# MVPandey/DTS

Measured on AMD Instinct MI355X. Metric: scored_trajectories_per_sec, higher is better.
Workload: dtype bf16

## Files before the change

dts_amd/models/llama.py:

```python

from __future__ import annotations

import math
from typing import Optional

import torch
import torch.nn as nn
import torch.nn.functional as F

from dts_amd import ops
from dts_amd.models.config import ModelSpec
from dts_amd.ops.torch_ref import build_rope_cache
from dts_amd.parallel.tp import (
    ColumnParallelLinear,
    RowParallelLinear,
    TPContext,
    _init_weight,
)
from dts_amd.serving.batch import ForwardBatch


class LlamaAttention(nn.Module):
    def __init__(self, spec: ModelSpec, tp: TPContext, dtype):
        super().__init__()
        self.tp = tp
        assert spec.num_heads % tp.size == 0
        assert spec.num_kv_heads % tp.size == 0 or tp.size % spec.num_kv_heads == 0
        self.num_heads = spec.num_heads // tp.size
        self.num_kv_heads = max(1, spec.num_kv_heads // tp.size)
        self.head_dim = spec.head_dim
        self.scale = 1.0 / math.sqrt(spec.head_dim)
        q_out = self.num_heads * self.head_dim * tp.size
        kv_out = self.num_kv_heads * self.head_dim * tp.size
        self.qkv_proj = ColumnParallelLinear(
            spec.hidden_size, q_out + 2 * kv_out, tp, dtype=dtype
        )
        self.o_proj = RowParallelLinear(
            self.num_heads * self.head_dim * tp.size, spec.hidden_size, tp, dtype=dtype
        )
        self.q_size = self.num_heads * self.head_dim
        self.kv_size = self.num_kv_heads * self.head_dim

    def forward(
        self,
        hidden: torch.Tensor,
        batch: ForwardBatch,
        kv_layer: tuple,
        rope: tuple,
    ) -> torch.Tensor:
        T = hidden.shape[0]
        qkv = self.qkv_proj(hidden)
        q, k, v = qkv.split([self.q_size, self.kv_size, self.kv_size], dim=-1)
        q = q.view(T, self.num_heads, self.head_dim)
        k = k.view(T, self.num_kv_heads, self.head_dim)
        v = v.view(T, self.num_kv_heads, self.head_dim)

        k_cache, v_cache = kv_layer
        cos, sin = rope
        q, k = ops.rope_kv_append(
            q, k, v, batch.positions, cos, sin, k_cache, v_cache, batch.slot_mapping
        )

        out = torch.empty(q.shape, dtype=q.dtype, device=q.device)
        np_tok = batch.num_prefill_tokens
        if batch.num_prefill_seqs:
            ops.attn_prefill_paged(
                q[:np_tok],
                batch.cu_q,
                batch.positions[:np_tok],
                k_cache,
                v_cache,
                batch.prefill_block_tables,
                batch.prefill_kv_lens,
                self.scale,
                out=out[:np_tok],
            )
        if batch.num_decode_seqs:
            ops.attn_decode_paged(
                q[np_tok:],
                k_cache,
                v_cache,
                batch.decode_block_tables,
                batch.decode_kv_lens,
                self.scale,
                out=out[np_tok:],
            )
        return self.o_proj(out.reshape(T, -1))


class LlamaMLP(nn.Module):
    def __init__(self, spec: ModelSpec, tp: TPContext, dtype):
        super().__init__()
        self.gate_up_proj = ColumnParallelLinear(
            spec.hidden_size, 2 * spec.intermediate_size, tp, dtype=dtype
# ... 132 lines not shown
```

dts_amd/ops/__init__.py:

```python

from __future__ import annotations

import os

import torch

from dts_amd.ops import torch_ref
from dts_amd.utils.logging import logger

_hip = None
_hip_load_error: Exception | None = None


def _try_load_hip():
    global _hip, _hip_load_error
    if _hip is not None or _hip_load_error is not None:
        return _hip
    try:
        from dts_amd.ops import _hip_ext_loader

        _hip = _hip_ext_loader.load()
        logger.info("HIP extension loaded: %s", _hip.__name__)
    except Exception as e:
        _hip_load_error = e
# ... 31 lines not shown
            ext.rmsnorm(out, x, weight, eps)
            return out
    return torch_ref.rmsnorm(x, weight, eps)


def fused_add_rmsnorm(x, residual, weight, eps=1e-5):
    if _on_gpu(x):
        ext = _require_hip()
        if ext is not None:
            ext.fused_add_rmsnorm(x, residual, weight, eps)
            return x, residual
    return torch_ref.fused_add_rmsnorm(x, residual, weight, eps)


def layernorm(x, weight, bias, eps=1e-5):
    if _on_gpu(x):
        ext = _require_hip()
        if ext is not None:
            out = torch.empty_like(x)
            ext.layernorm(out, x, weight, bias, eps)
            return out
    return torch_ref.layernorm(x, weight, bias, eps)


def rope_kv_append(q, k, v, positions, cos, sin, k_cache, v_cache, slot_mapping):
    if _on_gpu(q):
        ext = _require_hip()
        if ext is not None:
            ext.rope_kv_append(q, k, v, positions, cos, sin, k_cache, v_cache, slot_mapping)
            return q, k
    q, k = torch_ref.rope_apply(q, k, positions, cos, sin)
    torch_ref.kv_append(k, v, k_cache, v_cache, slot_mapping)
    return q, k


def kv_append(k, v, k_cache, v_cache, slot_mapping):
    if _on_gpu(k):
        ext = _require_hip()
        if ext is not None:
            ext.kv_append(k, v, k_cache, v_cache, slot_mapping)
            return
    torch_ref.kv_append(k, v, k_cache, v_cache, slot_mapping)


def attn_prefill_paged(
    q, cu_q, q_positions, k_cache, v_cache, block_tables, kv_lens, scale=None,
    out=None,
):
    if _on_gpu(q):
        ext = _require_hip()
        if ext is not None:
            import math

            if out is None or not out.is_contiguous():
                out = torch.empty(q.shape, dtype=q.dtype, device=q.device)
            ext.attn_prefill_paged(
                out, q, cu_q, q_positions, k_cache, v_cache, block_tables, kv_lens,
                scale if scale is not None else 1.0 / math.sqrt(q.shape[-1]),
            )
            return out
    ref = torch_ref.attn_prefill_paged(
        q, cu_q, q_positions, k_cache, v_cache, block_tables, kv_lens, scale
    )
    if out is not None:
        out.copy_(ref)
        return out
# ... 198 lines not shown
```

dts_amd/ops/hip/attention.hip:

```cpp

#include "common.h"
#include "kv_cache.h"
#include <torch/extension.h>
#include <c10/hip/HIPStream.h>
#include <unordered_map>
#include <array>
#include <cstdlib>

using bf16x8 = __attribute__((ext_vector_type(8))) short;
using f32x4 = __attribute__((ext_vector_type(4))) float;
using f32x2 = __attribute__((ext_vector_type(2))) float;
using bf16x2 = __attribute__((ext_vector_type(2))) __bf16;
using u32x2 = __attribute__((ext_vector_type(2))) unsigned int;
using u32x4 = __attribute__((ext_vector_type(4))) unsigned int;


DEV bf16x8 kv_deq8(u32x2 w) {
  union { bf16x2 p[4]; bf16x8 v; } c;
  c.p[0] = __builtin_amdgcn_cvt_scalef32_pk_bf16_fp8(w[0], 1.0f, false);
  c.p[1] = __builtin_amdgcn_cvt_scalef32_pk_bf16_fp8(w[0], 1.0f, true);
  c.p[2] = __builtin_amdgcn_cvt_scalef32_pk_bf16_fp8(w[1], 1.0f, false);
  c.p[3] = __builtin_amdgcn_cvt_scalef32_pk_bf16_fp8(w[1], 1.0f, true);
  return c.v;
}


template <int G, int D, typename KV = short>
__global__ void __launch_bounds__(256)
attn_decode_kernel(float* __restrict__ ws_m,
                   float* __restrict__ ws_l,
                   float* __restrict__ ws_o,
                   const short* __restrict__ q,
                   const KV* __restrict__ kcache,
                   const KV* __restrict__ vcache,
                   const int* __restrict__ block_tables,
                   const int* __restrict__ kv_lens,
                   int max_blocks, int Hkv, float scale, long q_tstride) {
  constexpr int BS = 16;
  constexpr int NWAVE = 4;
  constexpr int LPK = 4;
  constexpr int DPL = D / LPK;
  constexpr int DPV = D / WAVE;
  const int seq = blockIdx.x;
  const int kvh = blockIdx.y;
  const int split = blockIdx.z;
  const int S = gridDim.z;
  const int Hq = Hkv * G;
  const int wave = threadIdx.x / WAVE;
  const int lane = threadIdx.x & (WAVE - 1);
  const int kv_len = kv_lens[seq];
  const int n_pages = (kv_len + BS - 1) / BS;
  const int pages_per_split = (n_pages + S - 1) / S;
  const int page_lo = split * pages_per_split;
  const int page_hi = min(n_pages, page_lo + pages_per_split);
  const long ws_base = (((long)seq * Hkv + kvh) * S + split) * G;
  if (page_lo >= page_hi) {
    for (int g = threadIdx.x; g < G; g += blockDim.x) {
      ws_m[ws_base + g] = -1e30f;
      ws_l[ws_base + g] = 0.f;
    }
    return;
  }

  __shared__ float s_scores[NWAVE][G][BS];
  __shared__ float s_m[NWAVE][G], s_l[NWAVE][G];
  __shared__ float s_o[NWAVE][G][D];

  const int c = lane & (LPK - 1);
  const int key_of_lane = lane / LPK;
  int qp_[G][DPL / 2];
#pragma unroll
  for (int g = 0; g < G; ++g) {
    const short* qp = q + (long)seq * q_tstride + (long)(kvh * G + g) * D + c * DPL;
#pragma unroll
    for (int i = 0; i < DPL / 2; ++i) qp_[g][i] = ((const int*)qp)[i];
  }

  float m[G], lsum[G], o[G][DPV];
#pragma unroll
  for (int g = 0; g < G; ++g) {
    m[g] = -1e30f;
    lsum[g] = 0.f;
#pragma unroll
    for (int d = 0; d < DPV; ++d) o[g][d] = 0.f;
  }

  const int* bt = block_tables + (long)seq * max_blocks;

  for (int page = page_lo + wave; page < page_hi; page += NWAVE) {
    const long blk = bt[page];
    const KV* kbase =
        kcache + ((blk * Hkv + kvh) * BS) * (long)D;
    const KV* vbase =
// ... 121 lines not shown
  for (int g = 0; g < G; ++g) {
    if (lane == 0) {
      s_m[wave][g] = m[g];
      s_l[wave][g] = lsum[g];
    }
#pragma unroll
    for (int d = 0; d < DPV; ++d) s_o[wave][g][lane * DPV + d] = o[g][d];
  }
  __syncthreads();

  const int tid = threadIdx.x;
  for (int gd = tid; gd < G * (D / 2); gd += blockDim.x) {
    const int g = gd / (D / 2);
    const int d0 = (gd % (D / 2)) * 2;
    float m_star = -1e30f;
#pragma unroll
    for (int w = 0; w < NWAVE; ++w) m_star = fmaxf(m_star, s_m[w][g]);
    float l_star = 0.f, acc0 = 0.f, acc1 = 0.f;
#pragma unroll
    for (int w = 0; w < NWAVE; ++w) {
      float f = (s_m[w][g] > -1e30f) ? __expf(s_m[w][g] - m_star) : 0.f;
      l_star += s_l[w][g] * f;
      acc0 += s_o[w][g][d0] * f;
      acc1 += s_o[w][g][d0 + 1] * f;
    }
    if (d0 == 0) {
      ws_m[ws_base + g] = m_star;
      ws_l[ws_base + g] = l_star;
    }
    float* wo = ws_o + (ws_base + g) * D;
    wo[d0] = acc0;
    wo[d0 + 1] = acc1;
  }
}

template <int D>
__global__ void __launch_bounds__(256)
attn_decode_combine(short* __restrict__ out,
                    const float* __restrict__ ws_m,
                    const float* __restrict__ ws_l,
                    const float* __restrict__ ws_o,
                    int S, int G, int Hkv) {
  const int seq = blockIdx.x;
  const int hq = blockIdx.y;
  const int kvh = hq / G;
  const int g = hq % G;
  const int Hq = Hkv * G;
  const long base0 = (((long)seq * Hkv + kvh) * S) * G + g;

  __shared__ float sh_f[64];
  __shared__ float sh_linv[1];
  if (threadIdx.x == 0) {
    float m_star = -1e30f;
    for (int s2 = 0; s2 < S; ++s2)
      m_star = fmaxf(m_star, ws_m[base0 + (long)s2 * G]);
    float l_star = 0.f;
    for (int s2 = 0; s2 < S; ++s2) {
      float mm = ws_m[base0 + (long)s2 * G];
      float f = (mm > -1e30f) ? __expf(mm - m_star) : 0.f;
      sh_f[s2] = f;
      l_star += ws_l[base0 + (long)s2 * G] * f;
    }
    sh_linv[0] = (l_star > 0.f) ? 1.f / l_star : 0.f;
  }
  __syncthreads();
  const float linv = sh_linv[0];
// ... 695 lines not shown
    }
    __syncthreads();
  }

  {
    float invl[4];
#pragma unroll
    for (int i = 0; i < 4; ++i) {
      float l = s_rowl[wave][(lane >> 4) * 4 + i];
      invl[i] = (l > 0.f) ? 1.f / l : 0.f;
    }
#pragma unroll
    for (int ct = 0; ct < CTILES; ++ct) {
#pragma unroll
      for (int i = 0; i < 4; ++i) {
        const int row = (lane >> 4) * 4 + i;
        const int row_global = wave * 16 + row;
        const int pos_local = tile * POS_PER_WG + row_global / G;
        if (pos_local >= q_len) continue;
        const int head = row_global % G;
        const int tok = q_start + pos_local;
        const int dim = ct * 16 + (lane & 15);
        out[((long)tok * Hq + kvh * G + head) * D + dim] =
            f2bf(o_acc[ct][i] * invl[i]);
      }
    }
  }
}


void attn_decode_paged(torch::Tensor out, torch::Tensor q,
                       torch::Tensor kcache, torch::Tensor vcache,
                       torch::Tensor block_tables, torch::Tensor kv_lens,
                       double scale) {
  const int B = q.size(0), Hq = q.size(1), D = q.size(2);
  const int Hkv = kcache.size(1);
  const int G = Hq / Hkv;
  const int max_blocks = block_tables.size(1);
  TORCH_CHECK(kcache.size(2) == 16, "block_size must be 16");
  const bool fp8 = kv_cache_is_fp8(kcache, vcache);
  TORCH_CHECK(block_tables.scalar_type() == torch::kInt32);
  TORCH_CHECK(q.stride(2) == 1 && q.stride(1) == D, "q heads must be dense");
  TORCH_CHECK(out.is_contiguous(), "out must be contiguous");
  const long q_tstride = q.stride(0);
  static const int S = [] {
    const char* e = getenv("DTS_DECODE_SPLITS");
    int v = e ? atoi(e) : 8;
    return (v >= 1 && v <= 64) ? v : 8;
  }();
  static std::unordered_map<std::string, std::array<torch::Tensor, 3>> ws_cache;
  const std::string key = std::to_string(q.get_device()) + ":" +
                          std::to_string(B) + ":" + std::to_string(Hkv) + ":" +
                          std::to_string(G) + ":" + std::to_string(D);
  auto it = ws_cache.find(key);
  if (it == ws_cache.end()) {
    auto f32 =
        torch::TensorOptions().dtype(torch::kFloat32).device(q.device());
    it = ws_cache
             .emplace(key,
                      std::array<torch::Tensor, 3>{
                          torch::empty({B, Hkv, S, G}, f32),
                          torch::empty({B, Hkv, S, G}, f32),
                          torch::empty({(long)B, Hkv, S, G, D}, f32)})
             .first;
  }
  torch::Tensor ws_m = it->second[0];
  torch::Tensor ws_l = it->second[1];
  torch::Tensor ws_o = it->second[2];
  dim3 grid(B, Hkv, S);
  dim3 block(256);
  auto stream = c10::hip::getCurrentHIPStream();
#define DECODE_LAUNCH(g, d, kv)                                              \
  hipLaunchKernelGGL((attn_decode_kernel<g, d, kv>), grid, block, 0, stream, \
                     (float*)ws_m.data_ptr(), (float*)ws_l.data_ptr(),       \
                     (float*)ws_o.data_ptr(), (const short*)q.data_ptr(),    \
                     (const kv*)kcache.data_ptr(),                           \
                     (const kv*)vcache.data_ptr(),                           \
                     (const int*)block_tables.data_ptr(),                    \
                     (const int*)kv_lens.data_ptr(), max_blocks, Hkv,        \
                     (float)scale, q_tstride)
#define DECODE_CASE(g, d)                                                    \
  do {                                                                       \
    if (fp8) DECODE_LAUNCH(g, d, unsigned char);                             \
    else DECODE_LAUNCH(g, d, short);                                         \
    hipLaunchKernelGGL((attn_decode_combine<d>), dim3(B, Hq), dim3(256), 0,  \
                       stream, (short*)out.data_ptr(),                       \
                       (const float*)ws_m.data_ptr(),                        \
                       (const float*)ws_l.data_ptr(),                        \
                       (const float*)ws_o.data_ptr(), S, G, Hkv);            \
  } while (0)
  if (D == 128 && G == 4) DECODE_CASE(4, 128);
  else if (D == 128 && G == 8) DECODE_CASE(8, 128);
  else if (D == 128 && G == 1) DECODE_CASE(1, 128);
  else if (D == 64 && G == 1) DECODE_CASE(1, 64);
  else TORCH_CHECK(false, "unsupported decode attn shape D=", D, " G=", G);
#undef DECODE_CASE
#undef DECODE_LAUNCH
  HIP_CHECK_LAST();
}

void attn_prefill_paged(torch::Tensor out, torch::Tensor q, torch::Tensor cu_q,
                        torch::Tensor q_pos, torch::Tensor kcache,
                        torch::Tensor vcache, torch::Tensor block_tables,
                        torch::Tensor kv_lens, double scale, int64_t swz) {
  if (swz < 0) {
    static int env_v = [] {
      const char* e = getenv("DTS_PREFILL_V");
      return e ? atoi(e) : -1;
    }();
    swz = (env_v >= 0) ? env_v : 5;
  }
  const bool fp8 = kv_cache_is_fp8(kcache, vcache);
  TORCH_CHECK(!fp8 || swz == 0 || swz == 4 || swz == 5,
              "prefill variant ", swz, " (DTS_PREFILL_V) does not support an "
              "FP8 KV cache; use 0, 4 or 5");
  const int Hq = q.size(1), D = q.size(2);
  const int Hkv = kcache.size(1);
// ... 121 lines not shown
```

dts_amd/ops/hip/bindings.cpp:

```cpp
#include <torch/extension.h>

void rmsnorm(torch::Tensor out, torch::Tensor x, torch::Tensor w, double eps);
void fused_add_rmsnorm(torch::Tensor x, torch::Tensor residual,
                       torch::Tensor w, double eps);
void silu_mul(torch::Tensor out, torch::Tensor in);
void layernorm(torch::Tensor out, torch::Tensor x, torch::Tensor w,
               torch::Tensor b, double eps);
void rope_kv_append(torch::Tensor q, torch::Tensor k, torch::Tensor v,
                    torch::Tensor positions, torch::Tensor cos_t,
                    torch::Tensor sin_t, torch::Tensor k_cache,
                    torch::Tensor v_cache, torch::Tensor slots);
void kv_append(torch::Tensor k, torch::Tensor v, torch::Tensor k_cache,
               torch::Tensor v_cache, torch::Tensor slots);
void attn_decode_paged(torch::Tensor out, torch::Tensor q,
                       torch::Tensor kcache, torch::Tensor vcache,
                       torch::Tensor block_tables, torch::Tensor kv_lens,
                       double scale);
void attn_prefill_paged(torch::Tensor out, torch::Tensor q, torch::Tensor cu_q,
                        torch::Tensor q_pos, torch::Tensor kcache,
                        torch::Tensor vcache, torch::Tensor block_tables,
                        torch::Tensor kv_lens, double scale, int64_t swz);
void top_p_sample(torch::Tensor out, torch::Tensor logits, torch::Tensor temps,
                  torch::Tensor top_ps, torch::Tensor seeds);
void derive_seeds(torch::Tensor out, torch::Tensor bases,
                  torch::Tensor positions);
void top_p_sample_v2(torch::Tensor out, torch::Tensor logits,
                     torch::Tensor temps, torch::Tensor top_ps,
                     torch::Tensor seeds, torch::Tensor ws_max,
                     torch::Tensor ws_bins, torch::Tensor ws_slice,
                     torch::Tensor ws_tau);
void gemv_bf16(torch::Tensor out, torch::Tensor x, torch::Tensor w);
void gemm_skinny_bf16(torch::Tensor out, torch::Tensor x, torch::Tensor w,
                      int64_t tiles_per_wg, int64_t unroll);
void gemm_skinny_swiglu_bf16(torch::Tensor out, torch::Tensor x,
                             torch::Tensor w);
void moe_grouped_linear(torch::Tensor out, torch::Tensor x, torch::Tensor w,
                        torch::Tensor counts, torch::Tensor offsets);
void gemm_skinny_w8_bf16(torch::Tensor out, torch::Tensor x, torch::Tensor w_q,
                         torch::Tensor scale, int64_t tiles_per_wg,
                         int64_t unroll);
void gemm_skinny_swiglu_w8_bf16(torch::Tensor out, torch::Tensor x,
                                torch::Tensor w_q, torch::Tensor scale);

PYBIND11_MODULE(TORCH_EXTENSION_NAME, m) {
  m.def("rmsnorm", &rmsnorm, "RMSNorm (bf16, CDNA4)");
  m.def("fused_add_rmsnorm", &fused_add_rmsnorm,
        "fused residual add + RMSNorm (in-place, bf16)");
  m.def("silu_mul", &silu_mul, "SwiGLU activation (bf16)");
  m.def("layernorm", &layernorm, "LayerNorm (bf16, GPT-2 path)");
  m.def("rope_kv_append", &rope_kv_append,
        "fused rotate-half RoPE + paged KV append (bf16 q/k/v; bf16 or FP8 "
        "e4m3fn cache)");
  m.def("kv_append", &kv_append,
        "paged KV append without RoPE (bf16 k/v; bf16 or FP8 e4m3fn cache)");
  m.def("attn_decode_paged", &attn_decode_paged,
        "paged GQA decode attention (bf16 q/out, bf16 or FP8 e4m3fn cache)");
  m.def("attn_prefill_paged", &attn_prefill_paged,
        "paged causal prefill attention (bf16 MFMA; bf16 or FP8 e4m3fn cache)",
        py::arg("out"), py::arg("q"), py::arg("cu_q"), py::arg("q_pos"),
        py::arg("kcache"), py::arg("vcache"), py::arg("block_tables"),
        py::arg("kv_lens"),
        py::arg("scale"), py::arg("swz") = -1);
  m.def("top_p_sample", &top_p_sample,
        "fused temperature softmax + top-p sampling (sort-free)");
  m.def("derive_seeds", &derive_seeds,
        "stateless (seed, position) mix for chained decode");
  m.def("top_p_sample_v2", &top_p_sample_v2,
        "gridded top-p sampler (vocab sliced across workgroups)");
  m.def("gemv_bf16", &gemv_bf16,
        "skinny-batch (M<=8) bf16 weight-streaming GEMV");
  m.def("gemm_skinny_bf16", &gemm_skinny_bf16,
        "skinny-M (M<=16) bf16 MFMA weight-streaming GEMM; tiles_per_wg "
        "pins the N-tiles per workgroup (1/2/4), unroll the k-chunks in "
        "flight (4/8; 8 needs K % 1024 == 0); 0 = auto",
        py::arg("out"), py::arg("x"), py::arg("w"),
        py::arg("tiles_per_wg") = 0, py::arg("unroll") = 0);
  m.def("gemm_skinny_swiglu_bf16", &gemm_skinny_swiglu_bf16,
        "skinny-M gate_up GEMM with fused SwiGLU epilogue: "
        "out[M,I] = silu(x Wg^T) * (x Wu^T), w = [Wg; Wu]");
  m.def("moe_grouped_linear", &moe_grouped_linear,
        "grouped per-expert skinny GEMM (capture-safe MoE decode)");
  m.def("gemm_skinny_w8_bf16", &gemm_skinny_w8_bf16,
        "W8A16 skinny-M (M<=16) GEMM: FP8 e4m3fn weights [N,K] with an fp32 "
        "per-row scale [N], bf16 x/out, fp32 accumulation; tiles_per_wg and "
        "unroll as for gemm_skinny_bf16",
        py::arg("out"), py::arg("x"), py::arg("w_q"), py::arg("scale"),
        py::arg("tiles_per_wg") = 0, py::arg("unroll") = 0);
  m.def("gemm_skinny_swiglu_w8_bf16", &gemm_skinny_swiglu_w8_bf16,
        "W8A16 gate_up GEMM with fused SwiGLU epilogue: w_q = [Wg; Wu], "
        "gate rows scale by scale[n], up rows by scale[I+n]");
}
```

dts_amd/ops/hip/common.h:

```cpp
#pragma once

#include <hip/hip_runtime.h>
#include <hip/hip_bf16.h>
#include <hip/hip_fp16.h>

#define WAVE 64
#define DEV __device__ __forceinline__

typedef __attribute__((ext_vector_type(4))) short short4v;
typedef __attribute__((ext_vector_type(8))) short short8v;
typedef __attribute__((ext_vector_type(4))) float float4v;

DEV float bf2f(short u) {
  union { float f; unsigned int i; } c;
  c.i = ((unsigned int)(unsigned short)u) << 16;
  return c.f;
}

DEV short f2bf(float f) {
  union { float f; unsigned int i; } c;
  c.f = f;
  unsigned int lsb = (c.i >> 16) & 1;
  c.i += 0x7fff + lsb;
  return (short)(c.i >> 16);
}

DEV short swiglu_bf16(short gate, short up) {
  float gf = bf2f(gate);
  float s = gf / (1.f + __expf(-gf));
  return f2bf(s * bf2f(up));
}

DEV float wave_sum(float v) {
#pragma unroll
  for (int off = 32; off > 0; off >>= 1) v += __shfl_xor(v, off, 64);
  return v;
}

DEV float wave_max(float v) {
#pragma unroll
  for (int off = 32; off > 0; off >>= 1) v = fmaxf(v, __shfl_xor(v, off, 64));
  return v;
}

#define HIP_CHECK_LAST()                                                      \
  do {                                                                        \
    hipError_t e = hipGetLastError();                                         \
    if (e != hipSuccess) {                                                    \
      TORCH_CHECK(false, "HIP kernel launch failed: ", hipGetErrorString(e)); \
    }                                                                         \
  } while (0)
```

dts_amd/ops/hip/elementwise.hip:

```cpp

#include "common.h"
#include "kv_cache.h"
#include <torch/extension.h>
#include <c10/hip/HIPStream.h>


template <int BLOCK>
__global__ void rmsnorm_kernel(short* __restrict__ out,
                               const short* __restrict__ x,
                               const short* __restrict__ w, float eps, int T,
                               int H) {
  __shared__ float red[BLOCK / WAVE];
  for (int row = blockIdx.x; row < T; row += gridDim.x) {
    const short* xr = x + (long)row * H;
    short* yr = out + (long)row * H;
    float ss = 0.f;
    for (int i = threadIdx.x * 8; i < H; i += BLOCK * 8) {
      short8v v = *(const short8v*)(xr + i);
#pragma unroll
      for (int j = 0; j < 8; ++j) {
        float f = bf2f(v[j]);
        ss += f * f;
      }
    }
// ... 124 lines not shown
    short8v g = *(const short8v*)(in + t * 2 * I + i);
    short8v u = *(const short8v*)(in + t * 2 * I + I + i);
    short8v o;
#pragma unroll
    for (int j = 0; j < 8; ++j) o[j] = swiglu_bf16(g[j], u[j]);
    *(short8v*)(out + t * I + i) = o;
  }
}


template <typename KV>
__global__ void rope_kv_append_kernel(
    short* __restrict__ q, short* __restrict__ k, const short* __restrict__ v,
    const long* __restrict__ positions, const float* __restrict__ cos_t,
    const float* __restrict__ sin_t, KV* __restrict__ k_cache,
    KV* __restrict__ v_cache, const long* __restrict__ slots, int T, int Hq,
    int Hk, int D, int BS, long cache_head_stride, long cache_block_stride,
    int do_rope, long q_tstride, long k_tstride, long v_tstride) {
  int unit = blockIdx.x * (blockDim.x / WAVE) + threadIdx.x / WAVE;
  int lane = threadIdx.x & (WAVE - 1);
  int units = T * (Hq + 2 * Hk);
  if (unit >= units) return;
  int t = unit / (Hq + 2 * Hk);
  int h = unit % (Hq + 2 * Hk);
  long pos = positions[t];
  int half = D / 2;

  if (do_rope && h < Hq + Hk) {
    short* base = (h < Hq) ? q + (long)t * q_tstride + (long)h * D
                           : k + (long)t * k_tstride + (long)(h - Hq) * D;
    for (int i = lane; i < half; i += WAVE) {
      float c = cos_t[pos * half + i];
      float s = sin_t[pos * half + i];
      float x1 = bf2f(base[i]);
      float x2 = bf2f(base[i + half]);
      base[i] = f2bf(x1 * c - x2 * s);
      base[i + half] = f2bf(x2 * c + x1 * s);
    }
  }
  if (h >= Hq) {
    bool is_v = h >= Hq + Hk;
    int kvh = is_v ? (h - Hq - Hk) : (h - Hq);
    const short* src = is_v ? v + (long)t * v_tstride + (long)kvh * D
                            : k + (long)t * k_tstride + (long)kvh * D;
    KV* cache = is_v ? v_cache : k_cache;
    long slot = slots[t];
    long block = slot / BS, off = slot % BS;
    KV* dst = cache + block * cache_block_stride + kvh * cache_head_stride +
              off * D;
    if constexpr (sizeof(KV) == 1) {
      for (int i = lane * 4; i < D; i += WAVE * 4) {
        int w0 = *(const int*)(src + i);
        int w1 = *(const int*)(src + i + 2);
        auto sat = [](int u) {
          return fminf(fmaxf(bf2f((short)(u & 0xffff)), -448.f), 448.f);
        };
        float f0 = sat(w0), f1 = sat(w0 >> 16);
        float f2 = sat(w1), f3 = sat(w1 >> 16);
        int codes = __builtin_amdgcn_cvt_pk_fp8_f32(f0, f1, 0, false);
        codes = __builtin_amdgcn_cvt_pk_fp8_f32(f2, f3, codes, true);
        *(int*)(dst + i) = codes;
      }
    } else {
      for (int i = lane * 2; i < D; i += WAVE * 2) {
        *(int*)(dst + i) = *(const int*)(src + i);
      }
    }
  }
}

// ... 114 lines not shown
```

dts_amd/ops/hip/gemm_skinny.hip:

```cpp

#include "common.h"
#include <torch/extension.h>
#include <c10/hip/HIPStream.h>

using bf16x8 = __attribute__((ext_vector_type(8))) short;
using f32x4 = __attribute__((ext_vector_type(4))) float;

#define NWAVES 4
#define KSTEP 32
#define KUNROLL 4

template <int KU, int NT, bool SWIGLU>
__global__ void __launch_bounds__(NWAVES* WAVE)
gemm_skinny_kernel(short* __restrict__ out,
                   const short* __restrict__ x,
                   const short* __restrict__ w,
                   int M, int N, int K, long x_ts, long out_ts,
                   int wg_stride, int tile_stride) {
  static_assert(!SWIGLU || NT == 2, "SwiGLU pairs one gate and one up tile");
  const int wave = threadIdx.x / WAVE;
  const int lane = threadIdx.x & (WAVE - 1);
  const int n0 = blockIdx.x * wg_stride;

  const int kq = K / NWAVES;
  const int kbeg = wave * kq;
  const int kend = kbeg + kq;

  const int a_row = lane & 15;
  const int k_off = (lane >> 4) * 8;
  const bool a_live = a_row < M;
  const short* xrow = x + (long)a_row * x_ts;
  bool b_live[NT];
  const short* wrow[NT];
#pragma unroll
  for (int j = 0; j < NT; ++j) {
    const int b_row = n0 + j * tile_stride + (lane & 15);
    b_live[j] = b_row < N;
    wrow[j] = w + (long)(b_live[j] ? b_row : 0) * K;
  }

  f32x4 acc[NT];
#pragma unroll
  for (int j = 0; j < NT; ++j) acc[j] = {0.f, 0.f, 0.f, 0.f};
  const bf16x8 zero8 = {0, 0, 0, 0, 0, 0, 0, 0};

  auto load_group = [&](int k0, bf16x8 (&a)[KU], bf16x8 (&b)[NT][KU]) {
#pragma unroll
    for (int u = 0; u < KU; ++u) {
      const int kk = k0 + u * KSTEP + k_off;
      a[u] = a_live ? *(const bf16x8*)(xrow + kk) : zero8;
#pragma unroll
      for (int j = 0; j < NT; ++j)
        b[j][u] = b_live[j] ? *(const bf16x8*)(wrow[j] + kk) : zero8;
    }
  };
// ... 1 lines not shown
#pragma unroll
    for (int u = 0; u < KU; ++u)
#pragma unroll
      for (int j = 0; j < NT; ++j)
        acc[j] = __builtin_amdgcn_mfma_f32_16x16x32_bf16(a[u], b[j][u], acc[j],
                                                         0, 0, 0);
  };
  for (int k0 = kbeg; k0 < kend; k0 += KSTEP * KU) {
    bf16x8 a[KU], b[NT][KU];
    load_group(k0, a, b);
    mfma_group(a, b);
  }

  __shared__ float red[NT][NWAVES][16][16];
  const int c_col = lane & 15;
#pragma unroll
  for (int j = 0; j < NT; ++j)
#pragma unroll
    for (int i = 0; i < 4; ++i)
      red[j][wave][(lane >> 4) * 4 + i][c_col] = acc[j][i];
  __syncthreads();
  if constexpr (SWIGLU) {
    if (wave == 0) {
#pragma unroll
      for (int i = 0; i < 4; ++i) {
        const int m = (lane >> 4) * 4 + i;
        const int n = n0 + c_col;
        if (m < M && n < tile_stride) {
          float g = red[0][0][m][c_col] + red[0][1][m][c_col] +
                    red[0][2][m][c_col] + red[0][3][m][c_col];
          float u = red[1][0][m][c_col] + red[1][1][m][c_col] +
                    red[1][2][m][c_col] + red[1][3][m][c_col];
          out[(long)m * out_ts + n] = swiglu_bf16(f2bf(g), f2bf(u));
        }
      }
    }
  } else {
    for (int j = wave; j < NT; j += NWAVES) {
#pragma unroll
      for (int i = 0; i < 4; ++i) {
        const int m = (lane >> 4) * 4 + i;
        const int n = n0 + j * tile_stride + c_col;
        if (m < M && n < N) {
          float v = red[j][0][m][c_col] + red[j][1][m][c_col] +
                    red[j][2][m][c_col] + red[j][3][m][c_col];
          out[(long)m * out_ts + n] = f2bf(v);
        }
      }
    }
  }
}


__global__ void __launch_bounds__(NWAVES* WAVE)
moe_grouped_kernel(short* __restrict__ out,
                   const short* __restrict__ x,
                   const short* __restrict__ w,
                   const int* __restrict__ counts,
                   const int* __restrict__ offsets,
                   int N, int K) {
  const int wave = threadIdx.x / WAVE;
  const int lane = threadIdx.x & (WAVE - 1);
  const int n0 = blockIdx.x * 16;
  const int e = blockIdx.y;
  const int cnt = counts[e];
  if (cnt == 0) return;
// ... 49 lines not shown
}

void moe_grouped_linear(torch::Tensor out, torch::Tensor x, torch::Tensor w,
                        torch::Tensor counts, torch::Tensor offsets) {
  TORCH_CHECK(x.scalar_type() == torch::kBFloat16 && x.is_contiguous());
  TORCH_CHECK(w.is_contiguous(), "expert weights must be contiguous [E,N,K]");
  TORCH_CHECK(out.is_contiguous());
  TORCH_CHECK(counts.scalar_type() == torch::kInt32 &&
              offsets.scalar_type() == torch::kInt32);
  const int K = x.size(1), E = w.size(0), N = w.size(1);
  TORCH_CHECK(K % (NWAVES * KSTEP * KUNROLL) == 0, "K must be /512");
  const int tiles = (N + 15) / 16;
  hipLaunchKernelGGL(moe_grouped_kernel, dim3(tiles, E), dim3(NWAVES * WAVE),
                     0, c10::hip::getCurrentHIPStream(),
                     (short*)out.data_ptr(), (const short*)x.data_ptr(),
                     (const short*)w.data_ptr(),
                     (const int*)counts.data_ptr(),
                     (const int*)offsets.data_ptr(), N, K);
  HIP_CHECK_LAST();
}

static int skinny_unroll(int K, int64_t unroll) {
  static const int env_ku = [] {
    const char* e = getenv("DTS_SKINNY_UNROLL");
    return (e && e[0] == '8') ? 8 : (e && e[0] == '4') ? 4 : 0;
  }();
  TORCH_CHECK(unroll != 8 || K % (NWAVES * KSTEP * 8) == 0,
              "unroll=8 needs K % 1024 == 0, got K=", K);
  int ku = unroll ? (int)unroll : env_ku ? env_ku : (K >= 8192 ? 8 : 4);
  if (K % (NWAVES * KSTEP * 8) != 0) ku = 4;
  return ku;
}

#define SKINNY_LAUNCH(KU_, NT_, SW_, grid_, wgs_, ts_)                        \
  hipLaunchKernelGGL((gemm_skinny_kernel<KU_, NT_, SW_>), dim3(grid_),       \
                     dim3(NWAVES * WAVE), 0, stream, (short*)out.data_ptr(), \
                     (const short*)x.data_ptr(), (const short*)w.data_ptr(), \
                     M, N, K, x.stride(0), out.stride(0), wgs_, ts_)

static int skinny_auto_tiles(int M, int tiles) {
  if (M < 8) return 1;
  if (tiles >= 4096) return 4;
  if (tiles >= 1024) return M > 8 ? 4 : 1;
  if (tiles >= 384) return 2;
  return 1;
}

void gemm_skinny_bf16(torch::Tensor out, torch::Tensor x, torch::Tensor w,
                      int64_t tiles_per_wg, int64_t unroll) {
  TORCH_CHECK(x.scalar_type() == torch::kBFloat16);
  TORCH_CHECK(w.is_contiguous(), "weight must be contiguous [N, K]");
  TORCH_CHECK(x.stride(1) == 1, "x rows must be dense");
  TORCH_CHECK(out.stride(1) == 1);
  const int M = x.size(0), K = x.size(1), N = w.size(0);
  TORCH_CHECK(M >= 1 && M <= 16, "skinny path is for M<=16");
  TORCH_CHECK(K % (NWAVES * KSTEP * KUNROLL) == 0, "K must be /512");
  TORCH_CHECK(w.size(1) == K && out.size(0) == M && out.size(1) == N);
  TORCH_CHECK(tiles_per_wg == 0 || tiles_per_wg == 1 || tiles_per_wg == 2 ||
                  tiles_per_wg == 4,
              "tiles_per_wg must be 0 (auto), 1, 2 or 4");
  TORCH_CHECK(unroll == 0 || unroll == 4 || unroll == 8,
              "unroll must be 0 (auto), 4 or 8");
  const int tiles = (N + 15) / 16;
  const int nt =
      tiles_per_wg ? (int)tiles_per_wg : skinny_auto_tiles(M, tiles);
  const int grid = (tiles + nt - 1) / nt;
  auto stream = c10::hip::getCurrentHIPStream();
  if (skinny_unroll(K, unroll) == 8) {
    if (nt == 4) SKINNY_LAUNCH(8, 4, false, grid, 64, 16);
    else if (nt == 2) SKINNY_LAUNCH(8, 2, false, grid, 32, 16);
    else SKINNY_LAUNCH(8, 1, false, grid, 16, 16);
  } else {
    if (nt == 4) SKINNY_LAUNCH(4, 4, false, grid, 64, 16);
    else if (nt == 2) SKINNY_LAUNCH(4, 2, false, grid, 32, 16);
    else SKINNY_LAUNCH(4, 1, false, grid, 16, 16);
  }
  HIP_CHECK_LAST();
}

void gemm_skinny_swiglu_bf16(torch::Tensor out, torch::Tensor x,
                             torch::Tensor w) {
  TORCH_CHECK(x.scalar_type() == torch::kBFloat16);
  TORCH_CHECK(w.is_contiguous(), "weight must be contiguous [2I, K]");
  TORCH_CHECK(x.stride(1) == 1, "x rows must be dense");
  TORCH_CHECK(out.stride(1) == 1);
  const int M = x.size(0), K = x.size(1), N = w.size(0);
  const int I = N / 2;
  TORCH_CHECK(M >= 1 && M <= 16, "skinny path is for M<=16");
  TORCH_CHECK(K % (NWAVES * KSTEP * KUNROLL) == 0, "K must be /512");
  TORCH_CHECK(N == 2 * I && I % 16 == 0, "fused SwiGLU needs I % 16 == 0");
  TORCH_CHECK(w.size(1) == K && out.size(0) == M && out.size(1) == I);
  const int grid = I / 16;
  auto stream = c10::hip::getCurrentHIPStream();
  if (skinny_unroll(K, 0) == 8)
    SKINNY_LAUNCH(8, 2, true, grid, 16, I);
  else
    SKINNY_LAUNCH(4, 2, true, grid, 16, I);
  HIP_CHECK_LAST();
}
#undef SKINNY_LAUNCH
```

Before: 0.3880.

## Fuse QKV skinny GEMM with RoPE and paged KV append; add optional in-launch decode combine

For pure-decode batches with head_dim 128 and a bf16 cache, the QKV projection now runs a skinny GEMM variant whose epilogue applies rotate-half RoPE and writes K/V straight into the paged cache. This removes the separate rope_kv_append launch and its re-read of the qkv output. The change also adds an opt-in mode, off by default and enabled via an env var, that folds the split-KV decode combine into the decode kernel using an atomic ticket. The fused GEMM tiles heads as 128-wide pairs of 16-column tiles, so grid shape and per-block work differ from the plain skinny path.

```diff
diff --git a/dts_amd/models/llama.py b/dts_amd/models/llama.py
--- a/dts_amd/models/llama.py
+++ b/dts_amd/models/llama.py
@@ -49,17 +49,34 @@
         rope: tuple,
     ) -> torch.Tensor:
         T = hidden.shape[0]
-        qkv = self.qkv_proj(hidden)
+        k_cache, v_cache = kv_layer
+        cos, sin = rope
+        proj = self.qkv_proj
+        fused = (
+            proj.bias is None
+            and proj.weight_q is None
+            and not proj.gather_output
+            and ops.qkv_rope_fusable(
+                hidden, proj.weight, k_cache, self.num_heads, self.num_kv_heads,
+                self.head_dim, pure_decode=batch.num_prefill_seqs == 0,
+            )
+        )
+        if fused:
+            qkv = ops.linear_qkv_rope_append(
+                hidden, proj.weight, batch.positions, cos, sin, k_cache, v_cache,
+                batch.slot_mapping, self.num_heads, self.num_kv_heads,
+            )
+        else:
+            qkv = proj(hidden)
         q, k, v = qkv.split([self.q_size, self.kv_size, self.kv_size], dim=-1)
         q = q.view(T, self.num_heads, self.head_dim)
         k = k.view(T, self.num_kv_heads, self.head_dim)
         v = v.view(T, self.num_kv_heads, self.head_dim)
-
-        k_cache, v_cache = kv_layer
-        cos, sin = rope
-        q, k = ops.rope_kv_append(
-            q, k, v, batch.positions, cos, sin, k_cache, v_cache, batch.slot_mapping
-        )
+        if not fused:
+            q, k = ops.rope_kv_append(
+                q, k, v, batch.positions, cos, sin, k_cache, v_cache,
+                batch.slot_mapping,
+            )
 
         out = torch.empty(q.shape, dtype=q.dtype, device=q.device)
         np_tok = batch.num_prefill_tokens
diff --git a/dts_amd/ops/__init__.py b/dts_amd/ops/__init__.py
--- a/dts_amd/ops/__init__.py
+++ b/dts_amd/ops/__init__.py
@@ -87,6 +87,37 @@
     q, k = torch_ref.rope_apply(q, k, positions, cos, sin)
     torch_ref.kv_append(k, v, k_cache, v_cache, slot_mapping)
     return q, k
+
+
+def qkv_rope_fusable(
+    x, weight, k_cache, num_heads, num_kv_heads, head_dim, pure_decode=True
+) -> bool:
+    return (
+        pure_decode
+        and head_dim == 128
+        and os.environ.get("DTS_FUSED_QKV_ROPE") != "0"
+        and _skinny_kind(x, weight) == "skinny"
+        and weight.dtype == torch.bfloat16
+        and weight.is_contiguous()
+        and weight.shape[0] == (num_heads + 2 * num_kv_heads) * head_dim
+        and k_cache.dtype == torch.bfloat16
+        and hip_available()
+    )
+
+
+def linear_qkv_rope_append(
+    x, weight, positions, cos, sin, k_cache, v_cache, slot_mapping,
+    num_heads, num_kv_heads,
+):
+    ext = _require_hip()
+    if ext is None:
+        raise RuntimeError("linear_qkv_rope_append needs the HIP extension")
+    out = torch.empty((x.shape[0], weight.shape[0]), dtype=x.dtype, device=x.device)
+    ext.gemm_skinny_qkv_rope_append(
+        out, x, weight, positions, cos, sin, k_cache, v_cache, slot_mapping,
+        num_heads, num_kv_heads,
+    )
+    return out
 
 
 def kv_append(k, v, k_cache, v_cache, slot_mapping):
diff --git a/dts_amd/ops/hip/attention.hip b/dts_amd/ops/hip/attention.hip
--- a/dts_amd/ops/hip/attention.hip
+++ b/dts_amd/ops/hip/attention.hip
@@ -25,7 +25,87 @@
 }
 
 
-template <int G, int D, typename KV = short>
+template <int G, int D>
+DEV void decode_combine_tail(short* out,
+                             float* ws_m,
+                             float* ws_l, float* ws_o, int* cnt, int seq,
+                             int kvh, int Hkv, int S) {
+  __shared__ float t_f[G][64];
+  __shared__ float t_l[G][64];
+  __shared__ float t_linv[G];
+  __shared__ int t_last;
+  const int tid = threadIdx.x;
+  asm volatile("s_waitcnt vmcnt(0)" ::: "memory");
+  __syncthreads();
+  if (tid == 0) {
+    int* c = cnt + (long)seq * Hkv + kvh;
+    __builtin_amdgcn_fence(__ATOMIC_RELEASE, "agent");
+    asm volatile("s_waitcnt vmcnt(0)" ::: "memory");
+    const int ticket = __hip_atomic_fetch_add(c, 1, __ATOMIC_RELAXED,
+                                              __HIP_MEMORY_SCOPE_AGENT);
+    const int last = ticket == S - 1;
+    if (last) {
+      __hip_atomic_store(c, 0, __ATOMIC_RELAXED, __HIP_MEMORY_SCOPE_AGENT);
+      __builtin_amdgcn_fence(__ATOMIC_ACQUIRE, "agent");
+      asm volatile("s_waitcnt vmcnt(0)" ::: "memory");
+    }
+    t_last = last;
+  }
+  __syncthreads();
+  if (!t_last) return;
+
+  const long base0 = (((long)seq * Hkv + kvh) * S) * G;
+  for (int i = tid; i < S * G; i += blockDim.x) {
+    t_f[i % G][i / G] = ws_m[base0 + i];
+    t_l[i % G][i / G] = ws_l[base0 + i];
+  }
+  __syncthreads();
+  if (tid < G) {
+    const int g = tid;
+    float m_star = -1e30f;
+    for (int s2 = 0; s2 < S; ++s2) m_star = fmaxf(m_star, t_f[g][s2]);
+    float l_star = 0.f;
+    for (int s2 = 0; s2 < S; ++s2) {
+      float mm = t_f[g][s2];
+      float f = (mm > -1e30f) ? __expf(mm - m_star) : 0.f;
+      t_f[g][s2] = f;
+      l_star += t_l[g][s2] * f;
+    }
+    t_linv[g] = (l_star > 0.f) ? 1.f / l_star : 0.f;
+  }
+  __syncthreads();
+  const int Hq = Hkv * G;
+#pragma unroll 1
+  for (int it = tid; it < G * (D / 4); it += blockDim.x) {
+    const int g = it / (D / 4);
+    const int d0 = (it % (D / 4)) * 4;
+    const float linv = t_linv[g];
+    float4v acc = {0.f, 0.f, 0.f, 0.f};
+#pragma unroll 1
+    for (int s0 = 0; s0 < S; s0 += 8) {
+      float4v v[8];
+#pragma unroll
+      for (int u = 0; u < 8; ++u) {
+        const int s2 = min(s0 + u, S - 1);
+        v[u] = *(const float4v*)(ws_o + (base0 + (long)s2 * G + g) * D + d0);
+      }
+#pragma unroll
+      for (int u = 0; u < 8; ++u) {
+        const float f = (s0 + u < S) ? t_f[g][min(s0 + u, 63)] : 0.f;
+        if (f > 0.f) {
+#pragma unroll
+          for (int e = 0; e < 4; ++e) acc[e] += v[u][e] * f;
+        }
+      }
+    }
+    short4v o4;
+#pragma unroll
+    for (int e = 0; e < 4; ++e) o4[e] = f2bf(acc[e] * linv);
+    *(short4v*)(out + (((long)seq * Hq) + kvh * G + g) * D + d0) = o4;
+  }
+}
+
+template <int G, int D, typename KV = short, bool FUSED = false>
 __global__ void __launch_bounds__(256)
 attn_decode_kernel(float* __restrict__ ws_m,
                    float* __restrict__ ws_l,
@@ -35,7 +115,8 @@
                    const KV* __restrict__ vcache,
                    const int* __restrict__ block_tables,
                    const int* __restrict__ kv_lens,
-                   int max_blocks, int Hkv, float scale, long q_tstride) {
+                   int max_blocks, int Hkv, float scale, long q_tstride,
+                   short* out, int* cnt) {
   constexpr int BS = 16;
   constexpr int NWAVE = 4;
   constexpr int LPK = 4;
@@ -59,6 +140,8 @@
       ws_m[ws_base + g] = -1e30f;
       ws_l[ws_base + g] = 0.f;
     }
+    if constexpr (FUSED)
+      decode_combine_tail<G, D>(out, ws_m, ws_l, ws_o, cnt, seq, kvh, Hkv, S);
     return;
   }
 
@@ -246,6 +329,8 @@
     wo[d0] = acc0;
     wo[d0 + 1] = acc1;
   }
+  if constexpr (FUSED)
+    decode_combine_tail<G, D>(out, ws_m, ws_l, ws_o, cnt, seq, kvh, Hkv, S);
 }
 
 template <int D>
@@ -1007,7 +1092,7 @@
 void attn_decode_paged(torch::Tensor out, torch::Tensor q,
                        torch::Tensor kcache, torch::Tensor vcache,
                        torch::Tensor block_tables, torch::Tensor kv_lens,
-                       double scale) {
+                       double scale, int64_t fused) {
   const int B = q.size(0), Hq = q.size(1), D = q.size(2);
   const int Hkv = kcache.size(1);
   const int G = Hq / Hkv;
@@ -1017,13 +1102,20 @@
   TORCH_CHECK(block_tables.scalar_type() == torch::kInt32);
   TORCH_CHECK(q.stride(2) == 1 && q.stride(1) == D, "q heads must be dense");
   TORCH_CHECK(out.is_contiguous(), "out must be contiguous");
+  TORCH_CHECK(fused >= -1 && fused <= 1,
+              "fused must be -1 (auto), 0 (two kernels) or 1 (in-launch)");
   const long q_tstride = q.stride(0);
   static const int S = [] {
     const char* e = getenv("DTS_DECODE_SPLITS");
     int v = e ? atoi(e) : 8;
     return (v >= 1 && v <= 64) ? v : 8;
   }();
-  static std::unordered_map<std::string, std::array<torch::Tensor, 3>> ws_cache;
+  static const bool env_fused = [] {
+    const char* e = getenv("DTS_DECODE_FUSED_COMBINE");
+    return e && e[0] == '1';
+  }();
+  const bool use_fused = fused < 0 ? env_fused : fused == 1;
+  static std::unordered_map<std::string, std::array<torch::Tensor, 4>> ws_cache;
   const std::string key = std::to_string(q.get_device()) + ":" +
                           std::to_string(B) + ":" + std::to_string(Hkv) + ":" +
                           std::to_string(G) + ":" + std::to_string(D);
@@ -1033,31 +1125,40 @@
         torch::TensorOptions().dtype(torch::kFloat32).device(q.device());
     it = ws_cache
              .emplace(key,
-                      std::array<torch::Tensor, 3>{
+                      std::array<torch::Tensor, 4>{
                           torch::empty({B, Hkv, S, G}, f32),
                           torch::empty({B, Hkv, S, G}, f32),
-                          torch::empty({(long)B, Hkv, S, G, D}, f32)})
+                          torch::empty({(long)B, Hkv, S, G, D}, f32),
+                          torch::zeros({B, Hkv}, f32.dtype(torch::kInt32))})
              .first;
   }
   torch::Tensor ws_m = it->second[0];
   torch::Tensor ws_l = it->second[1];
   torch::Tensor ws_o = it->second[2];
+  torch::Tensor ws_cnt = it->second[3];
   dim3 grid(B, Hkv, S);
   dim3 block(256);
   auto stream = c10::hip::getCurrentHIPStream();
-#define DECODE_LAUNCH(g, d, kv)                                              \
-  hipLaunchKernelGGL((attn_decode_kernel<g, d, kv>), grid, block, 0, stream, \
-                     (float*)ws_m.data_ptr(), (float*)ws_l.data_ptr(),       \
-                     (float*)ws_o.data_ptr(), (const short*)q.data_ptr(),    \
+#define DECODE_LAUNCH(g, d, kv, fu)                                          \
+  hipLaunchKernelGGL((attn_decode_kernel<g, d, kv, fu>), grid, block, 0,     \
+                     stream, (float*)ws_m.data_ptr(),                        \
+                     (float*)ws_l.data_ptr(), (float*)ws_o.data_ptr(),       \
+                     (const short*)q.data_ptr(),                             \
                      (const kv*)kcache.data_ptr(),                           \
                      (const kv*)vcache.data_ptr(),                           \
                      (const int*)block_tables.data_ptr(),                    \
                      (const int*)kv_lens.data_ptr(), max_blocks, Hkv,        \
-                     (float)scale, q_tstride)
+                     (float)scale, q_tstride, (short*)out.data_ptr(),        \
+                     (int*)ws_cnt.data_ptr())
 #define DECODE_CASE(g, d)                                                    \
   do {                                                                       \
-    if (fp8) DECODE_LAUNCH(g, d, unsigned char);                             \
-    else DECODE_LAUNCH(g, d, short);                                         \
+    if (use_fused) {                                                         \
+      if (fp8) DECODE_LAUNCH(g, d, unsigned char, true);                     \
+      else DECODE_LAUNCH(g, d, short, true);                                 \
+      break;                                                                 \
+    }                                                                        \
+    if (fp8) DECODE_LAUNCH(g, d, unsigned char, false);                      \
+    else DECODE_LAUNCH(g, d, short, false);                                  \
     hipLaunchKernelGGL((attn_decode_combine<d>), dim3(B, Hq), dim3(256), 0,  \
                        stream, (short*)out.data_ptr(),                       \
                        (const float*)ws_m.data_ptr(),                        \
diff --git a/dts_amd/ops/hip/bindings.cpp b/dts_amd/ops/hip/bindings.cpp
--- a/dts_amd/ops/hip/bindings.cpp
+++ b/dts_amd/ops/hip/bindings.cpp
@@ -15,7 +15,7 @@
 void attn_decode_paged(torch::Tensor out, torch::Tensor q,
                        torch::Tensor kcache, torch::Tensor vcache,
                        torch::Tensor block_tables, torch::Tensor kv_lens,
-                       double scale);
+                       double scale, int64_t fused);
 void attn_prefill_paged(torch::Tensor out, torch::Tensor q, torch::Tensor cu_q,
                         torch::Tensor q_pos, torch::Tensor kcache,
                         torch::Tensor vcache, torch::Tensor block_tables,
@@ -34,6 +34,11 @@
                       int64_t tiles_per_wg, int64_t unroll);
 void gemm_skinny_swiglu_bf16(torch::Tensor out, torch::Tensor x,
                              torch::Tensor w);
+void gemm_skinny_qkv_rope_append(torch::Tensor out, torch::Tensor x,
+                                 torch::Tensor w, torch::Tensor positions,
+                                 torch::Tensor cos_t, torch::Tensor sin_t,
+                                 torch::Tensor k_cache, torch::Tensor v_cache,
+                                 torch::Tensor slots, int64_t Hq, int64_t Hk);
 void moe_grouped_linear(torch::Tensor out, torch::Tensor x, torch::Tensor w,
                         torch::Tensor counts, torch::Tensor offsets);
 void gemm_skinny_w8_bf16(torch::Tensor out, torch::Tensor x, torch::Tensor w_q,
@@ -54,7 +59,13 @@
   m.def("kv_append", &kv_append,
         "paged KV append without RoPE (bf16 k/v; bf16 or FP8 e4m3fn cache)");
   m.def("attn_decode_paged", &attn_decode_paged,
-        "paged GQA decode attention (bf16 q/out, bf16 or FP8 e4m3fn cache)");
+        "paged GQA decode attention (bf16 q/out, bf16 or FP8 e4m3fn cache); "
+        "fused: 1 = split-KV combine inside the decode launch, 0 = separate "
+        "combine kernel (default), -1 = auto (separate unless "
+        "DTS_DECODE_FUSED_COMBINE=1)",
+        py::arg("out"), py::arg("q"), py::arg("kcache"), py::arg("vcache"),
+        py::arg("block_tables"), py::arg("kv_lens"), py::arg("scale"),
+        py::arg("fused") = -1);
   m.def("attn_prefill_paged", &attn_prefill_paged,
         "paged causal prefill attention (bf16 MFMA; bf16 or FP8 e4m3fn cache)",
         py::arg("out"), py::arg("q"), py::arg("cu_q"), py::arg("q_pos"),
@@ -78,6 +89,13 @@
   m.def("gemm_skinny_swiglu_bf16", &gemm_skinny_swiglu_bf16,
         "skinny-M gate_up GEMM with fused SwiGLU epilogue: "
         "out[M,I] = silu(x Wg^T) * (x Wu^T), w = [Wg; Wu]");
+  m.def("gemm_skinny_qkv_rope_append", &gemm_skinny_qkv_rope_append,
+        "skinny-M fused qkv GEMM with rotate-half RoPE + paged KV append "
+        "epilogue (head_dim 128, bf16 cache): out and the caches end up as "
+        "gemm_skinny_bf16 + rope_kv_append leave them",
+        py::arg("out"), py::arg("x"), py::arg("w"), py::arg("positions"),
+        py::arg("cos"), py::arg("sin"), py::arg("k_cache"),
+        py::arg("v_cache"), py::arg("slots"), py::arg("Hq"), py::arg("Hk"));
   m.def("moe_grouped_linear", &moe_grouped_linear,
         "grouped per-expert skinny GEMM (capture-safe MoE decode)");
   m.def("gemm_skinny_w8_bf16", &gemm_skinny_w8_bf16,
diff --git a/dts_amd/ops/hip/common.h b/dts_amd/ops/hip/common.h
--- a/dts_amd/ops/hip/common.h
+++ b/dts_amd/ops/hip/common.h
@@ -31,6 +31,16 @@
   return f2bf(s * bf2f(up));
 }
 
+DEV void rope_rotate_bf16(short& a, short& b, float c, float s) {
+#pragma clang fp contract(off)
+  float x1 = bf2f(a);
+  float x2 = bf2f(b);
+  float x2s = x2 * s;
+  float x2c = x2 * c;
+  a = f2bf(__builtin_fmaf(x1, c, -x2s));
+  b = f2bf(__builtin_fmaf(x1, s, x2c));
+}
+
 DEV float wave_sum(float v) {
 #pragma unroll
   for (int off = 32; off > 0; off >>= 1) v += __shfl_xor(v, off, 64);
diff --git a/dts_amd/ops/hip/elementwise.hip b/dts_amd/ops/hip/elementwise.hip
--- a/dts_amd/ops/hip/elementwise.hip
+++ b/dts_amd/ops/hip/elementwise.hip
@@ -180,10 +180,11 @@
     for (int i = lane; i < half; i += WAVE) {
       float c = cos_t[pos * half + i];
       float s = sin_t[pos * half + i];
-      float x1 = bf2f(base[i]);
-      float x2 = bf2f(base[i + half]);
-      base[i] = f2bf(x1 * c - x2 * s);
-      base[i + half] = f2bf(x2 * c + x1 * s);
+      short x1 = base[i];
+      short x2 = base[i + half];
+      rope_rotate_bf16(x1, x2, c, s);
+      base[i] = x1;
+      base[i + half] = x2;
     }
   }
   if (h >= Hq) {
diff --git a/dts_amd/ops/hip/gemm_skinny.hip b/dts_amd/ops/hip/gemm_skinny.hip
--- a/dts_amd/ops/hip/gemm_skinny.hip
+++ b/dts_amd/ops/hip/gemm_skinny.hip
@@ -10,17 +10,34 @@
 #define KSTEP 32
 #define KUNROLL 4
 
-template <int KU, int NT, bool SWIGLU>
+enum { EPI_PLAIN = 0, EPI_SWIGLU = 1, EPI_QKV_ROPE = 2 };
+
+struct QkvRopeArgs {
+  const long* positions;
+  const float* cos_t;
+  const float* sin_t;
+  short* k_cache;
+  short* v_cache;
+  const long* slots;
+  int Hq, Hk, BS;
+  long cache_head_stride, cache_block_stride;
+};
+
+template <int KU, int NT, int EPI>
 __global__ void __launch_bounds__(NWAVES* WAVE)
 gemm_skinny_kernel(short* __restrict__ out,
                    const short* __restrict__ x,
                    const short* __restrict__ w,
                    int M, int N, int K, long x_ts, long out_ts,
-                   int wg_stride, int tile_stride) {
-  static_assert(!SWIGLU || NT == 2, "SwiGLU pairs one gate and one up tile");
+                   int wg_stride, int tile_stride, const QkvRopeArgs ra) {
+  constexpr bool SWIGLU = EPI == EPI_SWIGLU;
+  static_assert(EPI == EPI_PLAIN || NT == 2,
+                "the fused epilogues pair exactly two tiles");
   const int wave = threadIdx.x / WAVE;
   const int lane = threadIdx.x & (WAVE - 1);
-  const int n0 = blockIdx.x * wg_stride;
+  const int n0 = EPI == EPI_QKV_ROPE
+                     ? (blockIdx.x >> 2) * 128 + (blockIdx.x & 3) * 16
+                     : blockIdx.x * wg_stride;
 
   const int kq = K / NWAVES;
   const int kbeg = wave * kq;
@@ -88,6 +105,40 @@
           float u = red[1][0][m][c_col] + red[1][1][m][c_col] +
                     red[1][2][m][c_col] + red[1][3][m][c_col];
           out[(long)m * out_ts + n] = swiglu_bf16(f2bf(g), f2bf(u));
+        }
+      }
+    }
+  } else if constexpr (EPI == EPI_QKV_ROPE) {
+    if (wave == 0) {
+      const int h = blockIdx.x >> 2;
+      const int dim = (blockIdx.x & 3) * 16 + c_col;
+#pragma unroll
+      for (int i = 0; i < 4; ++i) {
+        const int m = (lane >> 4) * 4 + i;
+        if (m < M) {
+          short x1 = f2bf(red[0][0][m][c_col] + red[0][1][m][c_col] +
+                          red[0][2][m][c_col] + red[0][3][m][c_col]);
+          short x2 = f2bf(red[1][0][m][c_col] + red[1][1][m][c_col] +
+                          red[1][2][m][c_col] + red[1][3][m][c_col]);
+          if (h < ra.Hq + ra.Hk) {
+            const long pos = ra.positions[m];
+            rope_rotate_bf16(x1, x2, ra.cos_t[pos * 64 + dim],
+                             ra.sin_t[pos * 64 + dim]);
+          }
+          short* o = out + (long)m * out_ts + n0 + c_col;
+          o[0] = x1;
+          o[64] = x2;
+          if (h >= ra.Hq) {
+            const bool is_v = h >= ra.Hq + ra.Hk;
+            const int kvh = is_v ? h - ra.Hq - ra.Hk : h - ra.Hq;
+            const long slot = ra.slots[m];
+            const long block = slot / ra.BS, off = slot % ra.BS;
+            short* dst = (is_v ? ra.v_cache : ra.k_cache) +
+                         block * ra.cache_block_stride +
+                         kvh * ra.cache_head_stride + off * 128 + dim;
+            dst[0] = x1;
+            dst[64] = x2;
+          }
         }
       }
     }
@@ -203,11 +254,11 @@
   return ku;
 }
 
-#define SKINNY_LAUNCH(KU_, NT_, SW_, grid_, wgs_, ts_)                        \
-  hipLaunchKernelGGL((gemm_skinny_kernel<KU_, NT_, SW_>), dim3(grid_),       \
+#define SKINNY_LAUNCH(KU_, NT_, EPI_, grid_, wgs_, ts_, ra_)                  \
+  hipLaunchKernelGGL((gemm_skinny_kernel<KU_, NT_, EPI_>), dim3(grid_),      \
                      dim3(NWAVES * WAVE), 0, stream, (short*)out.data_ptr(), \
                      (const short*)x.data_ptr(), (const short*)w.data_ptr(), \
-                     M, N, K, x.stride(0), out.stride(0), wgs_, ts_)
+                     M, N, K, x.stride(0), out.stride(0), wgs_, ts_, ra_)
 
 static int skinny_auto_tiles(int M, int tiles) {
   if (M < 8) return 1;
@@ -237,14 +288,15 @@
       tiles_per_wg ? (int)tiles_per_wg : skinny_auto_tiles(M, tiles);
   const int grid = (tiles + nt - 1) / nt;
   auto stream = c10::hip::getCurrentHIPStream();
+  const QkvRopeArgs no_ra{};
   if (skinny_unroll(K, unroll) == 8) {
-    if (nt == 4) SKINNY_LAUNCH(8, 4, false, grid, 64, 16);
-    else if (nt == 2) SKINNY_LAUNCH(8, 2, false, grid, 32, 16);
-    else SKINNY_LAUNCH(8, 1, false, grid, 16, 16);
+    if (nt == 4) SKINNY_LAUNCH(8, 4, EPI_PLAIN, grid, 64, 16, no_ra);
+    else if (nt == 2) SKINNY_LAUNCH(8, 2, EPI_PLAIN, grid, 32, 16, no_ra);
+    else SKINNY_LAUNCH(8, 1, EPI_PLAIN, grid, 16, 16, no_ra);
   } else {
-    if (nt == 4) SKINNY_LAUNCH(4, 4, false, grid, 64, 16);
-    else if (nt == 2) SKINNY_LAUNCH(4, 2, false, grid, 32, 16);
-    else SKINNY_LAUNCH(4, 1, false, grid, 16, 16);
+    if (nt == 4) SKINNY_LAUNCH(4, 4, EPI_PLAIN, grid, 64, 16, no_ra);
+    else if (nt == 2) SKINNY_LAUNCH(4, 2, EPI_PLAIN, grid, 32, 16, no_ra);
+    else SKINNY_LAUNCH(4, 1, EPI_PLAIN, grid, 16, 16, no_ra);
   }
   HIP_CHECK_LAST();
 }
@@ -263,10 +315,63 @@
   TORCH_CHECK(w.size(1) == K && out.size(0) == M && out.size(1) == I);
   const int grid = I / 16;
   auto stream = c10::hip::getCurrentHIPStream();
+  const QkvRopeArgs no_ra{};
   if (skinny_unroll(K, 0) == 8)
-    SKINNY_LAUNCH(8, 2, true, grid, 16, I);
+    SKINNY_LAUNCH(8, 2, EPI_SWIGLU, grid, 16, I, no_ra);
   else
-    SKINNY_LAUNCH(4, 2, true, grid, 16, I);
+    SKINNY_LAUNCH(4, 2, EPI_SWIGLU, grid, 16, I, no_ra);
   HIP_CHECK_LAST();
 }
+
+void gemm_skinny_qkv_rope_append(torch::Tensor out, torch::Tensor x,
+                                 torch::Tensor w, torch::Tensor positions,
+                                 torch::Tensor cos_t, torch::Tensor sin_t,
+                                 torch::Tensor k_cache, torch::Tensor v_cache,
+                                 torch::Tensor slots, int64_t Hq, int64_t Hk) {
+  TORCH_CHECK(x.scalar_type() == torch::kBFloat16 &&
+              out.scalar_type() == torch::kBFloat16 &&
+              w.scalar_type() == torch::kBFloat16);
+  TORCH_CHECK(w.is_contiguous(), "weight must be contiguous [N, K]");
+  TORCH_CHECK(x.stride(1) == 1, "x rows must be dense");
+  TORCH_CHECK(out.stride(1) == 1);
+  const int M = x.size(0), K = x.size(1), N = w.size(0);
+  TORCH_CHECK(M >= 1 && M <= 16, "skinny path is for M<=16");
+  TORCH_CHECK(K % (NWAVES * KSTEP * KUNROLL) == 0, "K must be /512");
+  TORCH_CHECK(w.size(1) == K && out.size(0) == M && out.size(1) == N);
+  TORCH_CHECK(Hq >= 1 && Hk >= 1 && N == (Hq + 2 * Hk) * 128,
+              "fused qkv + RoPE needs head_dim 128 and N == (Hq+2Hk)*128");
+  TORCH_CHECK(positions.scalar_type() == torch::kInt64 &&
+              slots.scalar_type() == torch::kInt64 &&
+              positions.is_contiguous() && slots.is_contiguous() &&
+              positions.numel() == M && slots.numel() == M);
+  TORCH_CHECK(cos_t.scalar_type() == torch::kFloat32 &&
+              sin_t.scalar_type() == torch::kFloat32 &&
+              cos_t.is_contiguous() && sin_t.is_contiguous() &&
+              cos_t.size(-1) == 64 && sin_t.size(-1) == 64);
+  TORCH_CHECK(k_cache.scalar_type() == torch::kBFloat16 &&
+                  v_cache.scalar_type() == torch::kBFloat16,
+              "fused qkv + RoPE writes a bf16 cache only");
+  TORCH_CHECK(k_cache.dim() == 4 && k_cache.size(1) == Hk &&
+              k_cache.size(3) == 128 && k_cache.stride(3) == 1 &&
+              k_cache.stride(2) == 128 && v_cache.sizes() == k_cache.sizes() &&
+              v_cache.strides() == k_cache.strides());
+  const QkvRopeArgs ra{(const long*)positions.data_ptr(),
+                       (const float*)cos_t.data_ptr(),
+                       (const float*)sin_t.data_ptr(),
+                       (short*)k_cache.data_ptr(),
+                       (short*)v_cache.data_ptr(),
+                       (const long*)slots.data_ptr(),
+                       (int)Hq,
+                       (int)Hk,
+                       (int)k_cache.size(2),
+                       k_cache.stride(1),
+                       k_cache.stride(0)};
+  const int grid = (Hq + 2 * Hk) * 4;
+  auto stream = c10::hip::getCurrentHIPStream();
+  if (skinny_unroll(K, 0) == 8)
+    SKINNY_LAUNCH(8, 2, EPI_QKV_ROPE, grid, 0, 64, ra);
+  else
+    SKINNY_LAUNCH(4, 2, EPI_QKV_ROPE, grid, 0, 64, ra);
+  HIP_CHECK_LAST();
+}
 #undef SKINNY_LAUNCH
```

Measured after the change: 0.3905, median of 6. Within noise of the previous version (+0.7%).
